# bluecher31/mlff-preconditioner

Hardware: AMD Instinct MI355X
Metric: CG iters/sec + GB/s on N×N fp64 kernel mat-vec; iters-to-1e-6 vs CPU ref (higher is better)
Workload: dtype f64

## Files before the change

### mlff-preconditioner_amd/csrc/common.h

```cpp
#pragma once

#include <hip/hip_runtime.h>
#include <rccl/rccl.h>

#include <cstdint>
#include <memory>
#include <string>
#include <cstdlib>
#include <vector>

#include "../../include/mlffpcg.h"

namespace mlff {

constexpr int kWave = 64;
constexpr int kBlock = 256;
constexpr int kPad = 64;
constexpr int kMaxPart = 1024;
constexpr int kVecGrid = 512;
constexpr int kSymTile = 512;

__host__ __device__ inline int64_t round_up(int64_t a, int64_t b) { return (a + b - 1) / b * b; }

enum : int { ST_RUNNING = 0, ST_RECHECK = 1, ST_CONVERGED = 2, ST_MAXITER = 3, ST_FAULT = 4 };

struct DevState {
  double rho, rho1, alpha, pq, rr, resid, atol, pad0;
  long long iters;
  long long maxiter;
  int status;
  int linalg_err;
  int pivot_err;
  int pad1;
  long long m_pi;
  double sqrt_piv;
  double best_val;
  long long best_pos;
  double rho_new;
};

constexpr int kSymGenMaxD = 3;
constexpr double kSymStreamRate = 5600.0;
constexpr double kSymGenRate = 5600.0;
constexpr int kSymThreeWgMinUnits = 2;
struct SymGen {
  const double *Xs = nullptr;
  int d = 0;
  double jitter = 0.0;
  int64_t N = 0, rows_per = 0, blk = 0;
  int n_s = 0;
  int qmode = 0;
  int roles = 0;
  int pool_first = 0;
  int wgs = 2;
};
enum SymRoles : int { kSymRolesCu = 0, kSymRolesIndex = 1, kSymRolesStream = 2, kSymRolesGen = 3 };
constexpr int kSymCuWords = 4096;

struct SymPack {
  bool ready = false;
  double *tiles = nullptr;
  int2 *list = nullptr;
  int64_t ntiles = 0;
  int64_t Np = 0;
  int64_t nb = 0;
  int64_t tiles_per_rank = 0;
  double *P = nullptr;
  int64_t nwhole = 0;
  int lsub = 2;
  int64_t pq_planes = 0;
  double *Pq = nullptr;
  unsigned char *split = nullptr;
  int *own = nullptr;
  int *plist = nullptr;
  int64_t pstride = 0;
  int pmax = 0;
  bool pq_ordered = false;
  int64_t t_split = 0;
  int64_t dyn = 0;
  int wgs = 0;
  bool rb4 = false;
  unsigned long long *ticket = nullptr;
  bool gen = false;
  SymGen gsrc;
  double *yg = nullptr;
  double *yr = nullptr;
  int64_t ystride = 0;
};

constexpr int kSymOwnSplit = 1 << 24;
constexpr int kSymPlistSlotBits = 16;
constexpr int kSymPlistMaxSlots = (1 << kSymPlistSlotBits) - 1;
__host__ __device__ inline int sym_own_entry(int slot, bool split) {
  return slot | (split ? kSymOwnSplit : 0);
}
__host__ __device__ inline int sym_own_slot(int e) { return e & (kSymOwnSplit - 1); }
__host__ __device__ inline bool sym_own_split(int e) { return (e & kSymOwnSplit) != 0; }
__host__ __device__ inline int sym_plist_entry(int slot, int plane) {
  return slot | (plane << kSymPlistSlotBits);
}
__host__ __device__ inline int sym_plist_slot(int e) { return e & kSymPlistMaxSlots; }
__host__ __device__ inline int sym_plist_plane(int e) { return e >> kSymPlistSlotBits; }

struct MfData {
  bool ready = false;
  int64_t M = 0, D = 0;
  int n = 0, n_perms = 0;
  double sig = 0.0;
// ... 612 lines not shown
```

### mlff-preconditioner_amd/csrc/kernels_sym.hip

```cpp
#include "common.h"

#include <algorithm>
#include <cstdlib>
#include <cstring>

namespace mlff {

typedef double d2 __attribute__((ext_vector_type(2)));

namespace {

constexpr int B = kSymTile;
constexpr int kRB = 8;
constexpr int kBatches = B / kRB;
constexpr int kTileRed = 6 * B;
constexpr int kTileLds = kTileRed + 4 * kRB * 64;
constexpr int kGenRowLds = kSymGenMaxD * B + B / 64;

__device__ __forceinline__ void decode_unit(long long u, int nwhole, int lsub, int &tile, int &h,
                                            int &gb0, int &gb1) {
  if (u < nwhole) {
    tile = (int)u;
    h = 0;
    gb0 = 0;
// ... 4 lines not shown
    h = (int)(q & ((1 << lsub) - 1));
    gb0 = h * (kBatches >> lsub);
    gb1 = gb0 + (kBatches >> lsub);
  }
}

__device__ __forceinline__ double gathered_rho(const PGather &pg, double *sh) {
  double v = 0.0;
  const int np = pg.world * kVecGrid;
  int f = threadIdx.x;
  for (; f + 7 * 256 < np; f += 8 * 256) {
    double t[8];
#pragma unroll
    for (int u = 0; u < 8; ++u) {
      const int g = f + u * 256;
      t[u] = pg.gb[(int64_t)(g / kVecGrid) * pg.gstride + pg.blk + (g % kVecGrid)];
    }
#pragma unroll
    for (int u = 0; u < 8; ++u) v += t[u];
  }
  for (; f < np; f += 256) v += pg.gb[(int64_t)(f / kVecGrid) * pg.gstride + pg.blk + (f % kVecGrid)];
  v = block_sum256(v, sh);
  __syncthreads();
  if (threadIdx.x == 0) sh[4] = v;
  __syncthreads();
  const double rho = sh[4];
  __syncthreads();
  return rho;
}

__device__ __forceinline__ double pg_z(const PGather &pg, int64_t i) {
  const int64_t rk = i / pg.blk;
  return rk < pg.world ? pg.gb[rk * pg.gstride + i % pg.blk] : 0.0;
}
__device__ __forceinline__ double pg_val(const PGather &pg, const double *v, int64_t i, double beta) {
  return pg.it > 1 ? fma(beta, v[i], pg_z(pg, i)) : pg_z(pg, i);
}
__device__ __forceinline__ d2 pg_val2(const PGather &pg, const double *v, int64_t i, double beta) {
  if (pg.gb == nullptr) return *reinterpret_cast<const d2 *>(v + i);
  const int64_t rk = i / pg.blk;
  const d2 z = rk < pg.world ? *reinterpret_cast<const d2 *>(pg.gb + rk * pg.gstride + i % pg.blk)
                             : d2{0.0, 0.0};
  if (pg.it <= 1) return z;
  const d2 po = *reinterpret_cast<const d2 *>(v + i);
  return d2{fma(beta, po.x, z.x), fma(beta, po.y, z.y)};
}

__device__ __forceinline__ double fused_p_beta(const PGather &pg, double rho, double *publish) {
  const double beta = pg.it > 1 ? rho / pg.st->rho1 : 0.0;
  if (blockIdx.x == 0 && threadIdx.x == 0) *publish = rho;
  return beta;
}

constexpr int kTicketWords = 4;
__device__ __forceinline__ void reset_work_counters(unsigned long long *ticket) {
  ticket[0] = 0ull;
  ticket[2] = 0ull;
  ticket[3] = 0ull;
}

struct UnitQueue {
  unsigned long long *c0, *c1, *c2;
  long long base0, hi0, base1, hi1, base2, hi2;
  int stage;
};
__device__ __forceinline__ bool take_unit(unsigned long long *c, long long base, long long hi,
                                          long long &u) {
  if (base >= hi) return false;
  u = base + (long long)atomicAdd(c, 1ull);
  return u < hi;
}
__device__ __forceinline__ long long next_unit(UnitQueue &q, long long nunits) {
  long long u;
  if (q.stage == 0) {
    if (take_unit(q.c0, q.base0, q.hi0, u)) return u;
    q.stage = 1;
  }
  if (q.stage == 1) {
    if (take_unit(q.c1, q.base1, q.hi1, u)) return u;
    q.stage = 2;
  }
  if (q.stage == 2) {
    if (take_unit(q.c2, q.base2, q.hi2, u)) return u;
    q.stage = 3;
  }
  return nunits;
}

__device__ __forceinline__ bool gen_index(const SymGen &gs, int64_t pos, int64_t &g) {
  const int64_t off = pos % gs.blk;
  g = (pos / gs.blk) * gs.rows_per + off;
  return off < gs.rows_per && g < gs.N;
}

struct GenCols {
  double x[8][kSymGenMaxD];
  unsigned valid;
};
__device__ __forceinline__ void gen_load_cols(const SymGen &gs, int J, int lane, GenCols &gc) {
  gc.valid = 0u;
#pragma unroll
  for (int j = 0; j < 8; ++j) {
    int64_t g;
    const bool ok = gen_index(gs, (int64_t)J * B + 2 * (lane + 64 * (j >> 1)) + (j & 1), g);
    if (ok) gc.valid |= 1u << j;
#pragma unroll
    for (int t = 0; t < kSymGenMaxD; ++t) gc.x[j][t] = (ok && t < gs.d) ? gs.Xs[g * gs.d + t] : 0.0;
  }
}
__device__ __forceinline__ bool gen_row_inside(const double *xrow, int r) {
  const unsigned *mask = reinterpret_cast<const unsigned *>(xrow + kSymGenMaxD * B);
  return ((mask[r >> 5] >> (r & 31)) & 1u) != 0u;
}
__device__ __forceinline__ void gen_stage_rows(const SymGen &gs, int I, int r0, int nr,
                                               double *__restrict__ xrow) {
  unsigned *mask = reinterpret_cast<unsigned *>(xrow + kSymGenMaxD * B);
  for (int i = threadIdx.x; i < nr; i += 256) {
    int64_t g;
    const bool ok = gen_index(gs, (int64_t)I * B + r0 + i, g);
#pragma unroll
    for (int t = 0; t < kSymGenMaxD; ++t)
      xrow[kSymGenMaxD * (r0 + i) + t] = (ok && t < gs.d) ? gs.Xs[g * gs.d + t] : 0.0;
    const unsigned long long m = __ballot(ok);
    if ((threadIdx.x & 63) == 0) {
      mask[(r0 + i) >> 5] = (unsigned)m;
      if (nr - i > 32) mask[((r0 + i) >> 5) + 1] = (unsigned)(m >> 32);
    }
  }
}
__device__ __forceinline__ bool gen_block_full(const SymGen &gs, int Jb) {
  int64_t g;
  const int64_t p0 = (int64_t)Jb * B, p1 = p0 + B - 1;
  return p0 / gs.blk == p1 / gs.blk && gen_index(gs, p0, g) && gen_index(gs, p1, g);
}
template <bool PLAIN, bool DIAG>
__device__ __forceinline__ void gen_row(const SymGen &gs, const GenCols &gc,
                                        const double *__restrict__ xrow, int r, int lane,
                                        d2 (&ar)[4]) {
// ... 36 lines not shown

template <bool GEN, bool PLAIN, bool DIAG, int RB>
__device__ __forceinline__ void tile_batch(d2 (&a)[GEN ? 1 : RB][4], const double *A,
                                           const SymGen &gs,
                                           const GenCols &gc, const double *xrow,
                                           bool diag_rt, const d2 (&pc)[4],
                                           const double *vrow, int rbase, int lane,
                                           double *red, double *rows,
                                           d2 (&acc)[4]) {
  const bool diag = GEN ? DIAG : diag_rt;
#pragma unroll(GEN ? 2 : kRB)
  for (int rr = 0; rr < kRB; ++rr) {
    d2 ar[4];
    if constexpr (GEN) {
      gen_row<PLAIN, DIAG>(gs, gc, xrow, rbase + rr, lane, ar);
    } else {
      if constexpr (RB < kRB)
        if (rr == RB) tile_load_batch<RB>(A, rbase + RB, lane, a);
#pragma unroll
      for (int q = 0; q < 4; ++q) ar[q] = a[rr % RB][q];
    }
    double s0 = ar[0].x * pc[0].x;
    double s1 = ar[0].y * pc[0].y;
#pragma unroll
    for (int q = 1; q < 4; ++q) {
      s0 = fma(ar[q].x, pc[q].x, s0);
      s1 = fma(ar[q].y, pc[q].y, s1);
    }
    red[rr * 64 + lane] = s0 + s1;
    if (!diag) {
      const double pr = vrow[rbase + rr];
#pragma unroll
      for (int q = 0; q < 4; ++q) {
        acc[q].x = fma(ar[q].x, pr, acc[q].x);
        acc[q].y = fma(ar[q].y, pr, acc[q].y);
      }
    }
  }
  __builtin_amdgcn_fence(__ATOMIC_RELEASE, "wavefront");
  __builtin_amdgcn_wave_barrier();
  __builtin_amdgcn_fence(__ATOMIC_ACQUIRE, "wavefront");
  const d2 *rp = reinterpret_cast<const d2 *>(red + (lane >> 3) * 64 + (lane & 7) * 8);
  const d2 t0 = rp[0], t1 = rp[1], t2 = rp[2], t3 = rp[3];
  double tt = ((t0.x + t0.y) + (t1.x + t1.y)) + ((t2.x + t2.y) + (t3.x + t3.y));
  tt += __shfl_xor(tt, 1, 64);
  tt += __shfl_xor(tt, 2, 64);
  tt += __shfl_xor(tt, 4, 64);
  if ((lane & 7) == 0) rows[rbase + (lane >> 3)] = tt;
  __builtin_amdgcn_fence(__ATOMIC_RELEASE, "wavefront");
  __builtin_amdgcn_wave_barrier();
  __builtin_amdgcn_fence(__ATOMIC_ACQUIRE, "wavefront");
}

template <bool GEN, bool PLAIN, bool DIAG, int RB>
__device__ __forceinline__ void tile_batches(d2 (&a)[GEN ? 1 : RB][4], const double *A,
                                             const SymGen &gs, const GenCols &gc, const double *xrow,
                                             bool diag_rt, const d2 (&pc)[4], const double *vrow,
                                             int gb0, int gb1, int w, int lane, double *red,
                                             double *rows, d2 (&acc)[4]) {
#pragma unroll 1
  for (int g = gb0 + w; g < gb1; g += 4) {
    if constexpr (!GEN)
      if (g != gb0 + w) tile_load_batch<RB>(A, g * kRB, lane, a);
    tile_batch<GEN, PLAIN, DIAG, RB>(a, A, gs, gc, xrow, diag_rt, pc, vrow, g * kRB, lane, red, rows,
                                     acc);
  }
}
template <bool GEN, int RB>
__device__ __forceinline__ void tile_unit(d2 (&a)[GEN ? 1 : RB][4], const double *A,
                                          const SymGen &gs, const GenCols &gc, const double *xrow,
                                          bool plain, bool diag, const d2 (&pc)[4],
                                          const double *vrow, int gb0, int gb1, int w, int lane,
                                          double *red, double *rows, d2 (&acc)[4]) {
  if (GEN && plain)
    tile_batches<GEN, GEN, false, RB>(a, A, gs, gc, xrow, diag, pc, vrow, gb0, gb1, w, lane, red, rows, acc);
  else if (GEN && diag)
    tile_batches<GEN, false, GEN, RB>(a, A, gs, gc, xrow, diag, pc, vrow, gb0, gb1, w, lane, red, rows, acc);
  else
    tile_batches<GEN, false, false, RB>(a, A, gs, gc, xrow, diag, pc, vrow, gb0, gb1, w, lane, red, rows, acc);
}

__device__ __forceinline__ void tile_stage_cols(const d2 (&acc)[4], double *cs, int w, int lane) {
  d2 *cs2 = reinterpret_cast<d2 *>(cs);
#pragma unroll
  for (int q = 0; q < 4; ++q) cs2[w * (B / 2) + lane + 64 * q] = acc[q];
}

__device__ __forceinline__ void tile_store_slots(double *P, double *Pq,
                                                 int64_t Np, int nb, int2 t, int h, int gb0, int gb1,
                                                 bool diag, const double *sh) {
  const double *rows = sh + B, *cs = sh + 2 * B;
  const int row0 = gb0 * kRB, nr = (gb1 - gb0) * kRB;
  double *Prow = P + (int64_t)t.y * Np + (int64_t)t.x * B + row0;
  for (int c = threadIdx.x; c < nr; c += 256) __builtin_nontemporal_store(rows[row0 + c], Prow + c);
  if (!diag) {
    double *Pc = h == 0 ? P : Pq + (int64_t)(h - 1) * nb * Np;
    double *Pcol = Pc + (int64_t)t.x * Np + (int64_t)t.y * B;
    for (int c = threadIdx.x; c < B; c += 256)
      __builtin_nontemporal_store((cs[c] + cs[B + c]) + (cs[2 * B + c] + cs[3 * B + c]), Pcol + c);
  }
}

__global__ __launch_bounds__(256) void k_symv_tiles(const double *__restrict__ tiles,
                                                    const int2 *__restrict__ list,
                                                    const double *__restrict__ v,
                                                    double *__restrict__ P,
                                                    double *__restrict__ Pq, int64_t Np,
                                                    int nwhole, int nb, int lsub,
                                                    const int *__restrict__ status) {
  if (status != nullptr && *status != ST_RUNNING) return;
  __shared__ double sh[kTileLds];
  const int lane = threadIdx.x & 63, w = threadIdx.x >> 6;
  int tile, h, gb0, gb1;
  decode_unit(blockIdx.x, nwhole, lsub, tile, h, gb0, gb1);
  const int2 t = list[tile];
  const double *A = tiles + (int64_t)tile * B * B;
  d2 pc[4], a[kRB][4];
#pragma unroll
  for (int q = 0; q < 4; ++q)
    pc[q] = *reinterpret_cast<const d2 *>(v + (int64_t)t.y * B + 2 * (lane + 64 * q));
  tile_load_batch<kRB>(A, (int64_t)(gb0 + w) * kRB, lane, a);
  for (int i = gb0 * kRB + threadIdx.x; i < gb1 * kRB; i += 256) sh[i] = v[(int64_t)t.x * B + i];
  __syncthreads();
  const bool diag = t.x == t.y;
  const GenCols none{};
  d2 acc[4];
#pragma unroll
  for (int q = 0; q < 4; ++q) acc[q] = d2{0.0, 0.0};
  tile_unit<false, kRB>(a, A, SymGen{}, none, nullptr, false, diag, pc, sh, gb0, gb1, w, lane,
                   sh + kTileRed + w * kRB * 64, sh + B, acc);
  if (!diag) tile_stage_cols(acc, sh + 2 * B, w, lane);
  __syncthreads();
  tile_store_slots(P, Pq, Np, nb, t, h, gb0, gb1, diag, sh);
}

struct SymvArgs {
  const double *tiles;
  const int2 *list;
  const double *v;
  double *P, *Pq;
  int64_t Np;
  int nwhole;
  long long nunits;
  int nb, lsub;
  PGather pg;
  double beta;
};

template <bool GEN, int RB>
__device__ __forceinline__ long long symv_units(const SymvArgs &k, const SymGen &gs, long long u,
                                                UnitQueue q, double *__restrict__ sh,
                                                long long *s_next) {
  const int lane = threadIdx.x & 63, w = threadIdx.x >> 6;
  double *vrow = sh, *rows = sh + B, *cs = sh + 2 * B;
  double *red = sh + kTileRed + w * kRB * 64;
  double *xrow = sh + kTileLds;
  const PGather &pg = k.pg;
  const double *v = k.v;
  const double beta = k.beta;
  long long units_done = 0;
  int tile, h, gb0, gb1;
  decode_unit(u, k.nwhole, k.lsub, tile, h, gb0, gb1);
  int2 t = k.list[tile];
  const double *A = k.tiles + (int64_t)tile * B * B;
  d2 pc[4], a[GEN ? 1 : RB][4];
  GenCols gc;
#pragma unroll
  for (int q = 0; q < 4; ++q) pc[q] = pg_val2(pg, v, (int64_t)t.y * B + 2 * (lane + 64 * q), beta);
  if constexpr (!GEN) tile_load_batch<RB>(A, (int64_t)(gb0 + w) * kRB, lane, a);
  if (threadIdx.x == 0) *s_next = next_unit(q, k.nunits);
  for (int i = threadIdx.x; i < (gb1 - gb0) * kRB; i += 256) {
    const int64_t gi = (int64_t)t.x * B + gb0 * kRB + i;
    vrow[gb0 * kRB + i] = pg.gb != nullptr ? pg_val(pg, v, gi, beta) : v[gi];
  }
  if (GEN) {
    gen_stage_rows(gs, t.x, gb0 * kRB, (gb1 - gb0) * kRB, xrow);
    gen_load_cols(gs, t.y, lane, gc);
  }
  __syncthreads();
  while (true) {
    const bool diag = t.x == t.y;
    const bool plain = GEN && !diag && gen_block_full(gs, t.x) && gen_block_full(gs, t.y);
    d2 acc[4];
#pragma unroll
    for (int q = 0; q < 4; ++q) acc[q] = d2{0.0, 0.0};
    tile_unit<GEN, RB>(a, A, gs, gc, xrow, plain, diag, pc, vrow, gb0, gb1, w, lane, red, rows, acc);
    if (!diag) tile_stage_cols(acc, cs, w, lane);
    __syncthreads();
    const long long un = *s_next;
    int tile2 = 0, h2 = 0, gb02 = 0, gb12 = 0;
    int2 t2 = t;
    const double *A2 = A;
    if (un < k.nunits) {
      decode_unit(un, k.nwhole, k.lsub, tile2, h2, gb02, gb12);
      t2 = k.list[tile2];
      A2 = k.tiles + (int64_t)tile2 * B * B;
#pragma unroll
      for (int q = 0; q < 4; ++q)
        pc[q] = pg_val2(pg, v, (int64_t)t2.y * B + 2 * (lane + 64 * q), beta);
      if constexpr (GEN)
        gen_load_cols(gs, t2.y, lane, gc);
      else
        tile_load_batch<RB>(A2, (int64_t)(gb02 + w) * kRB, lane, a);
    }
    tile_store_slots(k.P, k.Pq, k.Np, k.nb, t, h, gb0, gb1, diag, sh);
    __syncthreads();
    ++units_done;
    if (un >= k.nunits) break;
    if (threadIdx.x == 0) *s_next = next_unit(q, k.nunits);
    tile = tile2;
    h = h2;
    gb0 = gb02;
    gb1 = gb12;
    t = t2;
    A = A2;
    for (int i = threadIdx.x; i < (gb1 - gb0) * kRB; i += 256) {
      const int64_t gi = (int64_t)t.x * B + gb0 * kRB + i;
      vrow[gb0 * kRB + i] = pg.gb != nullptr ? pg_val(pg, v, gi, beta) : v[gi];
    }
    if (GEN) gen_stage_rows(gs, t.x, gb0 * kRB, (gb1 - gb0) * kRB, xrow);
    __syncthreads();
  }
  return units_done;
}

__device__ __forceinline__ unsigned cu_key() {
  unsigned xcc = 0, hw = 0;
  asm volatile("s_getreg_b32 %0, hwreg(HW_REG_XCC_ID)" : "=s"(xcc));
  asm volatile("s_getreg_b32 %0, hwreg(HW_REG_HW_ID)" : "=s"(hw));
  return ((xcc & 0xfu) << 8) | ((hw >> 8) & 0xffu);
}

constexpr int kTraceWords = 4;

template <bool ROLES, int RB = kRB>
__global__ __launch_bounds__(256, RB < kRB ? 3 : 1) void k_symv_dyn(const double *__restrict__ tiles,
                                                  const int2 *__restrict__ list,
                                                  const double *__restrict__ v,
                                                  double *__restrict__ P,
                                                  double *__restrict__ Pq, int64_t Np,
                                                  int nwhole, long long nunits, int nb,
                                                  int lsub,
                                                  unsigned long long *__restrict__ ticket,
                                                  const int *__restrict__ status, PGather pg,
                                                  SymGen gs,
                                                  unsigned long long *wgtrace = nullptr) {
  if (status != nullptr && *status != ST_RUNNING) return;
  unsigned long long *tr = wgtrace != nullptr ? wgtrace + kTraceWords * blockIdx.x : nullptr;
  if (tr != nullptr && threadIdx.x == 0) tr[0] = wall_clock64();
  __shared__ double sh[kTileLds + (ROLES ? kGenRowLds : 0)];
  __shared__ long long s_next;
  __shared__ int s_role;
  if (!ROLES && (long long)blockIdx.x >= nunits) return;
  if (ROLES && threadIdx.x == 0) {
    int r = gs.roles == kSymRolesGen ? 1 : 0;
    const unsigned wgs = (unsigned)gs.wgs;
    if (gs.roles == kSymRolesIndex) r = blockIdx.x % wgs != 0u;
    if (gs.roles == kSymRolesCu) r = atomicAdd(ticket + kTicketWords + cu_key(), 1ull) % wgs != 0ull;
    s_role = r;
  }
  if (!ROLES && tr != nullptr && threadIdx.x == 0) tr[3] = 1ull | (unsigned long long)cu_key() << 2;
  const double beta = pg.gb != nullptr ? fused_p_beta(pg, gathered_rho(pg, sh), &pg.st->rho_new) : 0.0;
  UnitQueue q{ticket, ticket, ticket, (long long)gridDim.x, nunits, 0, 0, 0, 0, 0};
  long long u = blockIdx.x;
  bool gen = false;
  if (ROLES) {
    __syncthreads();
    gen = __builtin_amdgcn_readfirstlane(s_role) != 0;
    const bool pool_first = gs.pool_first != 0 && gs.qmode != (gen ? 1 : 2);
    unsigned long long *cs = ticket, *cg = ticket + 2, *cq = ticket + 3;
    const long long ns = gs.n_s;
    q.c0 = gen ? cg : cs;
    q.base0 = gen ? ns : 0;
    q.hi0 = gen ? nwhole : ns;
    unsigned long long *co = gen ? cs : cg;
    const long long olo = gen ? 0 : ns, ohi = gen ? ns : nwhole;
    q.c1 = pool_first ? cq : co;
    q.base1 = pool_first ? nwhole : olo;
    q.hi1 = pool_first ? nunits : ohi;
    q.c2 = pool_first ? co : cq;
    q.base2 = pool_first ? olo : nwhole;
    q.hi2 = pool_first ? ohi : nunits;
    if (threadIdx.x == 0) {
      s_next = next_unit(q, nunits);
      if (tr != nullptr) tr[3] = 1ull | (gen ? 2ull : 0ull) | (unsigned long long)cu_key() << 2;
    }
    __syncthreads();
    u = s_next;
    __syncthreads();
    if (u >= nunits) {
      if (tr != nullptr && threadIdx.x == 0) tr[1] = wall_clock64();
      return;
    }
  }
  const SymvArgs k{tiles, list, v, P, Pq, Np, nwhole, nunits, nb, lsub, pg, beta};
  long long units_done;
  if constexpr (ROLES) {
    if (gen)
      units_done = symv_units<true, RB>(k, gs, u, q, sh, &s_next);
    else
      units_done = symv_units<false, RB>(k, gs, u, q, sh, &s_next);
  } else {
    units_done = symv_units<false, RB>(k, gs, u, q, sh, &s_next);
  }
  if (tr != nullptr && threadIdx.x == 0) {
    tr[1] = wall_clock64();
    tr[2] = (unsigned long long)units_done;
  }
}

template <bool EPI, bool PQ>
__global__ __launch_bounds__(256) void k_sym_reduce(const double *__restrict__ P,
                                                    const double *__restrict__ Pq,
                                                    const unsigned char *__restrict__ split,
                                                    int t_split, int64_t Np, int nb, int nq,
                                                    int64_t n_out, double *__restrict__ y,
                                                    double sigma, double lam,
                                                    const double *__restrict__ vloc,
                                                    double *__restrict__ pq_part,
                                                    unsigned long long *__restrict__ ticket,
                                                    const int *__restrict__ status,
                                                    PGather pg = PGather{},
                                                    double *pw = nullptr) {
  if (status != nullptr && *status != ST_RUNNING) return;
  if (blockIdx.x == 0 && threadIdx.x == 0) reset_work_counters(ticket);
  double apq = 0.0;
  const double beta = PQ && pg.gb != nullptr ? fused_p_beta(pg, pg.st->rho_new, &pg.st->rho) : 0.0;
  const int64_t pl = (int64_t)nb * Np;
  for (int64_t i = (int64_t)blockIdx.x * 256 + threadIdx.x; i < n_out;
       i += (int64_t)gridDim.x * 256) {
    const int bi = (int)(i / B);
    double s = 0.0;
    const int tend = t_split > bi ? t_split : bi + 1;
    const int t8 = tend < nb ? tend : nb;
    int t = 0;
    for (; t + 15 < t8; t += 16) {
      double v[16];
#pragma unroll
      for (int u = 0; u < 16; ++u) v[u] = __builtin_nontemporal_load(P + (int64_t)(t + u) * Np + i);
#pragma unroll
      for (int u = 0; u < 16; ++u) s += v[u];
    }
    for (; t + 7 < t8; t += 8) {
      double v[8];
#pragma unroll
      for (int u = 0; u < 8; ++u) v[u] = __builtin_nontemporal_load(P + (int64_t)(t + u) * Np + i);
#pragma unroll
      for (int u = 0; u < 8; ++u) s += v[u];
    }
    for (; t < nb; t += 8) {
      double v[8];
#pragma unroll
      for (int u = 0; u < 8; ++u) {
        v[u] = 0.0;
        const int tu = t + u;
        if (tu < nb) {
          v[u] = P[(int64_t)tu * Np + i];
          if (tu > bi && split[(int64_t)tu * nb + bi])
            for (int hq = 0; hq < nq; ++hq) v[u] += Pq[hq * pl + (int64_t)tu * Np + i];
// ... 345 lines not shown
  int64_t gc[2];
  bool vc[2];
#pragma unroll
  for (int h = 0; h < 2; ++h) {
    const int64_t pos = (int64_t)t.y * B + threadIdx.x + 256 * h;
    const int64_t off = pos % blk;
    gc[h] = (pos / blk) * rows_per + off;
    vc[h] = off < rows_per && gc[h] < N;
#pragma unroll
    for (int u = 0; u < 8; ++u) xc[h][u] = (vc[h] && u < d) ? Xs[gc[h] * d + u] : 0.0;
  }
  for (int r = 0; r < B; ++r) {
    const int64_t pos = (int64_t)t.x * B + r;
    const int64_t off = pos % blk;
    const int64_t gr = (pos / blk) * rows_per + off;
    const bool vr = off < rows_per && gr < N;
#pragma unroll
    for (int h = 0; h < 2; ++h) {
      double val = 0.0;
      if (vr && vc[h]) val = (gr == gc[h]) ? 1.0 + jitter : rbf_value(xc[h], Xs, gr, d);
      __builtin_nontemporal_store(val, T + (int64_t)r * B + threadIdx.x + 256 * h);
    }
  }
}

__global__ __launch_bounds__(256) void k_rbf_exp_probe(const double *__restrict__ s, int64_t n,
                                                       double *__restrict__ lib_out,
                                                       double *__restrict__ lean_out) {
  for (int64_t i = (int64_t)blockIdx.x * 256 + threadIdx.x; i < n; i += (int64_t)gridDim.x * 256) {
    lib_out[i] = rbf_of_sqdist(s[i]);
    lean_out[i] = rbf_of_sqdist_lean(s[i]);
  }
}

}

void launch_rbf_exp_probe(const double *s, int64_t n, double *lib_out, double *lean_out,
                          hipStream_t st) {
  if (n <= 0) return;
  const unsigned grid = (unsigned)std::min<int64_t>((n + 255) / 256, 4096);
  hipLaunchKernelGGL(k_rbf_exp_probe, dim3(grid), dim3(256), 0, st, s, n, lib_out, lean_out);
}

struct SymKnobs {
  int64_t whole_rounds = -1;
  int lsub = 2;
  bool dynamic = true;
  bool gen = true;
  int64_t gen_tiles = -1;
  int gen_quarters = 0;
  int roles = kSymRolesCu;
  int pool_first = 0;
  int wgs = 0;
  bool reduce_list = true;
  bool pq_ordered = false;
  long long trace_at = 0;
};

static SymKnobs sym_knobs() {
  SymKnobs k;
  if (const char *e = std::getenv("MLFF_SYM_WHOLE_ROUNDS")) k.whole_rounds = std::max<int64_t>(0, std::atoll(e));
  if (const char *e = std::getenv("MLFF_SYM_LSUB")) {
    const int v = std::atoi(e);
    if (v >= 1 && v <= 4) k.lsub = v;
  }
  if (const char *e = std::getenv("MLFF_SYM_SCHED")) k.dynamic = std::strcmp(e, "static") != 0;
  if (const char *e = std::getenv("MLFF_SYM_GEN")) k.gen = std::atoi(e) != 0;
  if (const char *e = std::getenv("MLFF_SYM_GEN_TILES")) k.gen_tiles = std::max<int64_t>(0, std::atoll(e));
  if (const char *e = std::getenv("MLFF_SYM_GEN_QUARTERS")) {
    const int v = std::atoi(e);
    if (v >= 0 && v <= 2) k.gen_quarters = v;
  }
  if (const char *e = std::getenv("MLFF_SYM_ROLES")) {
    if (std::strcmp(e, "index") == 0) k.roles = kSymRolesIndex;
    if (std::strcmp(e, "stream") == 0) k.roles = kSymRolesStream;
    if (std::strcmp(e, "gen") == 0) k.roles = kSymRolesGen;
  }
  if (const char *e = std::getenv("MLFF_SYM_STEAL")) k.pool_first = std::strcmp(e, "pool") == 0;
  if (const char *e = std::getenv("MLFF_SYM_WGS")) {
    const int v = std::atoi(e);
    if (v == 2 || v == 3) k.wgs = v;
  }
  if (const char *e = std::getenv("MLFF_SYM_REDUCE_LIST")) k.reduce_list = std::atoi(e) != 0;
  if (const char *e = std::getenv("MLFF_SYM_PQ_ORDERED")) k.pq_ordered = std::atoi(e) != 0;
  if (const char *e = std::getenv("MLFF_SYM_TRACE")) k.trace_at = std::atoll(e);
  return k;
}

static void print_symv_trace(const unsigned long long *tr, unsigned G, int64_t units, int wgs,
                             hipStream_t s) {
  std::vector<unsigned long long> h((size_t)kTraceWords * G);
  if (hipStreamSynchronize(s) != hipSuccess ||
      hipMemcpy(h.data(), tr, sizeof(unsigned long long) * h.size(), hipMemcpyDeviceToHost) != hipSuccess)
    return;
  unsigned long long t0 = ~0ull, t1 = 0;
  std::vector<double> st, en, un;
  for (unsigned g = 0; g < G; ++g) {
    const unsigned long long *r = &h[(size_t)kTraceWords * g];
    if (r[0] == 0) continue;
    t0 = std::min(t0, r[0]);
    t1 = std::max(t1, r[1]);
  }
  double idle = 0.0;
  std::vector<int> cu_s(kSymCuWords, 0), cu_g(kSymCuWords, 0);
  int xs[16] = {0}, xg[16] = {0};
  double un_s = 0.0, un_g = 0.0;
  for (unsigned g = 0; g < G; ++g) {
    const unsigned long long *r = &h[(size_t)kTraceWords * g];
    if (r[0] == 0) continue;
    st.push_back(10.0 * (double)(r[0] - t0));
    en.push_back(10.0 * (double)(r[1] - t0));
    un.push_back((double)r[2]);
    idle += 10.0 * (double)(t1 - r[1]) + 10.0 * (double)(r[0] - t0);
    if (!(r[3] & 1ull)) continue;
    const bool gen = (r[3] & 2ull) != 0;
    const unsigned key = (unsigned)(r[3] >> 2) & (kSymCuWords - 1);
    ++(gen ? cu_g : cu_s)[key];
    ++(gen ? xg : xs)[key >> 8];
    (gen ? un_g : un_s) += (double)r[2];
  }
  auto q = [](std::vector<double> v, double f) {
    std::sort(v.begin(), v.end());
    return v.empty() ? 0.0 : v[(size_t)(f * (double)(v.size() - 1))];
  };
  const double span = 10.0 * (double)(t1 - t0);
  std::fprintf(stderr,
               "[sym trace] units %lld on %zu workgroups (units per wg p0/p50/p100 %.0f/%.0f/%.0f); "
               "span %.1f us; starts p50/p100 %.1f/%.1f us; ends p0/p10/p50/p90/p100 "
               "%.1f/%.1f/%.1f/%.1f/%.1f us; idle (ramp + tail) %.1f %% of wg-time\n",
               (long long)units, st.size(), q(un, 0.0), q(un, 0.5), q(un, 1.0), 1e-3 * span,
               1e-3 * q(st, 0.5), 1e-3 * q(st, 1.0), 1e-3 * q(en, 0.0), 1e-3 * q(en, 0.1),
               1e-3 * q(en, 0.5), 1e-3 * q(en, 0.9), 1e-3 * q(en, 1.0),
               100.0 * idle / (span * (double)st.size()));
  int cus = 0, paired = 0, two_s = 0, two_g = 0, other = 0;
  for (int k = 0; k < kSymCuWords; ++k) {
    if (cu_s[k] + cu_g[k] == 0) continue;
    ++cus;
    if (cu_s[k] == 1 && cu_g[k] == wgs - 1)
      ++paired;
    else if (cu_s[k] == wgs && cu_g[k] == 0)
      ++two_s;
    else if (cu_s[k] == 0 && cu_g[k] == wgs)
      ++two_g;
    else
      ++other;
  }
  std::string per_xcc;
  for (int x = 0; x < 16; ++x)
    if (xs[x] + xg[x] > 0)
      per_xcc += " " + std::to_string(x) + ":" + std::to_string(xs[x]) + "s+" + std::to_string(xg[x]) + "g";
  std::fprintf(stderr,
               "[sym trace] roles: %d distinct CU keys; CUs holding {1 stream + %d gen} %d, {%d stream} "
               "%d, {%d gen} %d, other %d; units taken stream / gen %.0f / %.0f (%.0f / %.0f per ms "
               "of the span); per XCC id%s\n",
               cus, wgs - 1, paired, wgs, two_s, wgs, two_g, other, un_s, un_g, 1e6 * un_s / span,
               1e6 * un_g / span, per_xcc.c_str());
}

void launch_symv(const SymPack &sp, const double *v_full, double *P, const int *status,
                 hipStream_t s, PGather pg) {
  if (sp.ntiles == 0) return;
  const int64_t grid = sp.nwhole + ((sp.ntiles - sp.nwhole) << sp.lsub);
  if (sp.dyn == 0) {
    hipLaunchKernelGGL(k_symv_tiles, dim3((unsigned)grid), dim3(256), 0, s, sp.tiles, sp.list, v_full,
                       P, sp.Pq, sp.Np, (int)sp.nwhole, (int)sp.nb, sp.lsub, status);
    return;
  }
  const unsigned G = (unsigned)std::min<int64_t>(sp.dyn, grid);
  static const long long trace_at = sym_knobs().trace_at;
  static long long launches = 0;
  unsigned long long *tr = nullptr;
  if (trace_at > 0 && ++launches == trace_at &&
      hipMalloc(&tr, sizeof(unsigned long long) * kTraceWords * G) == hipSuccess)
    (void)hipMemsetAsync(tr, 0, sizeof(unsigned long long) * kTraceWords * G, s);
  if (sp.gen && sp.rb4)
    hipLaunchKernelGGL((k_symv_dyn<true, 4>), dim3(G), dim3(256), 0, s,
                       sp.tiles, sp.list, v_full, P, sp.Pq, sp.Np, (int)sp.nwhole, (long long)grid,
                       (int)sp.nb, sp.lsub, sp.ticket, status, pg, sp.gsrc, tr);
  else if (sp.gen)
    hipLaunchKernelGGL(k_symv_dyn<true>, dim3(G), dim3(256), 0, s,
                       sp.tiles, sp.list, v_full, P, sp.Pq, sp.Np, (int)sp.nwhole, (long long)grid,
                       (int)sp.nb, sp.lsub, sp.ticket, status, pg, sp.gsrc, tr);
  else
    hipLaunchKernelGGL(k_symv_dyn<false>, dim3(G), dim3(256), 0, s,
                       sp.tiles, sp.list, v_full, P, sp.Pq, sp.Np, (int)sp.nwhole, (long long)grid,
                       (int)sp.nb, sp.lsub, sp.ticket, status, pg, SymGen{}, tr);
// ... 77 lines not shown
  const int a = I / tpr, c = J / tpr;
  if (a == c) return a;
  return ((I + J) & 1) ? a : c;
}


struct SymPlan {
  int64_t Np = 0;
  int nb = 0, tpr = 0;
  std::vector<int2> list;
  std::vector<unsigned char> trans;
  int64_t nt = 0, nwhole = 0;
  int lsub = 2;
  int64_t nq = 3;
  int64_t dyn = 0;
  int wgs = 2;
  bool rb4 = false;
  bool gen = false;
  SymGen gsrc;
};

static SymPlan sym_plan(const mlff_ctx *ctx, const SymKnobs &kn) {
  SymPlan pl;
  pl.Np = round_up(ctx->ld, B);
  pl.nb = (int)(pl.Np / B);
  pl.tpr = ctx->world > 1 ? (int)(ctx->blk / B) : pl.nb;
  for (int I = 0; I < pl.nb; ++I)
    for (int J = 0; J <= I; ++J) {
      if (owner_host(I, J, pl.tpr) != ctx->rank) continue;
      pl.list.push_back(make_int2(I, J));
      pl.trans.push_back(ctx->world > 1 && (I / pl.tpr) != ctx->rank ? 1 : 0);
    }
  pl.nt = (int64_t)pl.list.size();
  int cus = 0;
  if (hipDeviceGetAttribute(&cus, hipDeviceAttributeMultiprocessorCount, ctx->device) != hipSuccess ||
      cus < 1)
    cus = 256;
  const int64_t C = 2 * (int64_t)cus;
  pl.nwhole = (pl.nt / C) * C;
  if (kn.whole_rounds >= 0) pl.nwhole = std::min<int64_t>(pl.nwhole, kn.whole_rounds * C);
  pl.lsub = kn.lsub;
  pl.nq = ((int64_t)1 << pl.lsub) - 1;
  pl.dyn = kn.dynamic ? C : 0;
  if (pl.dyn > 0 && pl.nt > 0 && !ctx->has_matrix && ctx->rbf.ready && ctx->rbf.d >= 1 &&
      ctx->rbf.d <= kSymGenMaxD) {
    int64_t n_s = (int64_t)((double)pl.nwhole * kSymStreamRate / (kSymStreamRate + kSymGenRate) + 0.5);
    if (kn.gen_tiles >= 0) n_s = pl.nwhole - std::min<int64_t>(pl.nwhole, kn.gen_tiles);
    const int qmode = kn.gen_quarters;
    bool on = kn.gen;
    if (pl.nwhole == pl.nt && n_s == pl.nwhole) on = false;
    if (n_s == pl.nwhole && qmode == 1) on = false;
    if (on) {
      pl.gen = true;
      if (kn.wgs != 2) {
        int occ = 0;
        if (hipOccupancyMaxActiveBlocksPerMultiprocessor(&occ, k_symv_dyn<true, 4>, 256, 0) != hipSuccess ||
            occ < 1)
          occ = 2;
        const int64_t nunits = pl.nwhole + ((pl.nt - pl.nwhole) << pl.lsub);
        pl.rb4 = kn.wgs == 3 || (occ > 2 && nunits >= kSymThreeWgMinUnits * occ * cus);
        if (pl.rb4) {
          pl.wgs = occ;
          pl.dyn = (int64_t)occ * cus;
        }
      }
      pl.gsrc = SymGen{ctx->rbf.Xs, ctx->rbf.d, ctx->rbf.jitter, ctx->N, ctx->rows_per, ctx->blk,
                       (int)n_s, qmode, kn.roles, kn.pool_first, pl.wgs};
    }
  }
  return pl;
}

static int sym_alloc(mlff_ctx *ctx, const SymPlan &pl, const SymKnobs &kn) {
  SymPack &sp = ctx->sym;
  hipStream_t s = ctx->stream;
  const int64_t nt = pl.nt, nb = pl.nb, Np = pl.Np, nq = pl.nq;
  if (sp.tiles == nullptr || sp.ntiles != nt || sp.Np != Np || sp.pq_planes != nq) {
    sym_free(sp);
    if (nt > 0) {
      MLFF_HIP(ctx, hipMalloc(&sp.tiles, sizeof(double) * nt * B * B));
      MLFF_HIP(ctx, hipMalloc(&sp.list, sizeof(int2) * nt));
    }
    MLFF_HIP(ctx, hipMalloc(&sp.P, sizeof(double) * nb * Np));
    MLFF_HIP(ctx, hipMemsetAsync(sp.P, 0, sizeof(double) * nb * Np, s));
    MLFF_HIP(ctx, hipMalloc(&sp.Pq, sizeof(double) * nq * nb * Np));
    MLFF_HIP(ctx, hipMemsetAsync(sp.Pq, 0, sizeof(double) * nq * nb * Np, s));
    sp.pq_planes = nq;
    MLFF_HIP(ctx, hipMalloc(&sp.split, (size_t)nb * nb));
    MLFF_HIP(ctx, hipMalloc(&sp.own, sizeof(int) * (size_t)nb * (nb + 1)));
    const size_t tw = (kTicketWords + kSymCuWords) * sizeof(unsigned long long);
    MLFF_HIP(ctx, hipMalloc(&sp.ticket, tw));
    MLFF_HIP(ctx, hipMemsetAsync(sp.ticket, 0, tw, s));
    if (ctx->world > 1) {
      sp.ystride = ctx->blk + round_up(ctx->world, kPad);
      const int64_t ny = (int64_t)ctx->world * sp.ystride;
      MLFF_HIP(ctx, hipMalloc(&sp.yg, sizeof(double) * ny));
      MLFF_HIP(ctx, hipMalloc(&sp.yr, sizeof(double) * sp.ystride));
      MLFF_HIP(ctx, hipMemsetAsync(sp.yg, 0, sizeof(double) * ny, s));
      MLFF_HIP(ctx, hipMemsetAsync(sp.yr, 0, sizeof(double) * sp.ystride, s));
    }
  }
  sp.ntiles = nt;
  sp.Np = Np;
  sp.nb = nb;
  sp.tiles_per_rank = pl.tpr;
  sp.nwhole = pl.nwhole;
  sp.lsub = pl.lsub;
  sp.dyn = pl.dyn;
  sp.wgs = pl.dyn > 0 ? pl.wgs : 0;
  sp.rb4 = pl.rb4;
  sp.gen = pl.gen;
  sp.gsrc = pl.gsrc;
  sp.pq_ordered = kn.pq_ordered;
  return MLFF_OK;
}

static int sym_slot_tables(mlff_ctx *ctx, const SymPlan &pl, const SymKnobs &kn) {
  SymPack &sp = ctx->sym;
  hipStream_t s = ctx->stream;
  const int nb = pl.nb;
// ... 101 lines not shown
```

Before: 625.1.

## Defer next-unit claim to last batch and lower three-workgroup threshold

The dynamic symmetric mat-vec scheduler now claims its next work unit late, during the final batch of the current tile, instead of at tile start. This keeps units from being reserved early by workgroups that will not reach them for a while, which should reduce tail imbalance. It also lowers the unit-count threshold for switching to three workgroups per CU when late commit is on, and adds an optional endgame rule (off by default) where generator workgroups decline whole tiles near the end. A per-wave lambda call and extra trace instrumentation are added; the late claim may expose atomic latency at the tile boundary.

```diff
diff --git a/mlff-preconditioner_amd/csrc/common.h b/mlff-preconditioner_amd/csrc/common.h
--- a/mlff-preconditioner_amd/csrc/common.h
+++ b/mlff-preconditioner_amd/csrc/common.h
@@ -7,6 +7,7 @@
 #include <memory>
 #include <string>
 #include <cstdlib>
+#include <cstring>
 #include <vector>
 
 #include "../../include/mlffpcg.h"
@@ -42,7 +43,7 @@
 constexpr int kSymGenMaxD = 3;
 constexpr double kSymStreamRate = 5600.0;
 constexpr double kSymGenRate = 5600.0;
-constexpr int kSymThreeWgMinUnits = 2;
+constexpr double kSymThreeWgMinUnits = 1.375;
 struct SymGen {
   const double *Xs = nullptr;
   int d = 0;
@@ -53,7 +54,27 @@
   int roles = 0;
   int pool_first = 0;
   int wgs = 2;
-};
+  int late = 0;
+  int endgame = 0;
+};
+constexpr double kSymEndgameRounds = 0.0;
+constexpr bool kSymLateCommit = true;
+inline void sym_parse_commit(const char *e, bool &late) {
+  if (e == nullptr) return;
+  if (std::strcmp(e, "early") == 0) late = false;
+  if (std::strcmp(e, "late") == 0) late = true;
+}
+inline void sym_parse_endgame(const char *e, double &rounds) {
+  if (e == nullptr) return;
+  char *end = nullptr;
+  const double v = std::strtod(e, &end);
+  if (end != e && v >= 0.0 && v <= 1e9) rounds = v;
+}
+inline int sym_endgame_theta(double rounds, int64_t workgroups, int wgs) {
+  if (!(rounds > 0.0) || wgs < 1) return 0;
+  const double t = rounds * (double)(workgroups / wgs) + 0.5;
+  return t >= 2147483647.0 ? 2147483647 : (int)t;
+}
 enum SymRoles : int { kSymRolesCu = 0, kSymRolesIndex = 1, kSymRolesStream = 2, kSymRolesGen = 3 };
 constexpr int kSymCuWords = 4096;
 
diff --git a/mlff-preconditioner_amd/csrc/kernels_sym.hip b/mlff-preconditioner_amd/csrc/kernels_sym.hip
--- a/mlff-preconditioner_amd/csrc/kernels_sym.hip
+++ b/mlff-preconditioner_amd/csrc/kernels_sym.hip
@@ -80,17 +80,25 @@
   return beta;
 }
 
-constexpr int kTicketWords = 4;
+constexpr int kTicketWords = 6;
+constexpr int kTicketPresent = 4;
 __device__ __forceinline__ void reset_work_counters(unsigned long long *ticket) {
   ticket[0] = 0ull;
   ticket[2] = 0ull;
   ticket[3] = 0ull;
-}
+  ticket[kTicketPresent] = 0ull;
+}
+
+constexpr int kTraceWords = 10;
+enum : int { kTrEmpty = 4, kTrDecline = 5, kTrLast = 6, kTrCyc0 = 7, kTrCyc1 = 8, kTrDry = 9 };
 
 struct UnitQueue {
   unsigned long long *c0, *c1, *c2;
   long long base0, hi0, base1, hi1, base2, hi2;
   int stage;
+  const unsigned long long *ticket;
+  int theta;
+  unsigned long long *tr;
 };
 __device__ __forceinline__ bool take_unit(unsigned long long *c, long long base, long long hi,
                                           long long &u) {
@@ -98,20 +106,40 @@
   u = base + (long long)atomicAdd(c, 1ull);
   return u < hi;
 }
+__device__ __forceinline__ unsigned long long counter_now(const unsigned long long *c) {
+  return __hip_atomic_load(c, __ATOMIC_RELAXED, __HIP_MEMORY_SCOPE_AGENT);
+}
+__device__ __forceinline__ bool endgame_declines(const UnitQueue &q) {
+  if (q.theta <= 0 || q.stage > 2) return false;
+  if (counter_now(q.ticket + kTicketPresent) == 0ull) return false;
+  const unsigned long long ts = counter_now(q.ticket), tg = counter_now(q.ticket + 2);
+  const long long n_s = q.base0, n_g = q.hi0 - q.base0;
+  const long long left = (n_s - (long long)min(ts, (unsigned long long)n_s)) +
+                         (n_g - (long long)min(tg, (unsigned long long)n_g));
+  return left <= q.theta;
+}
+__device__ __forceinline__ void trace_once(unsigned long long *tr, int word) {
+  if (tr != nullptr && tr[word] == 0ull) tr[word] = wall_clock64();
+}
+__device__ __forceinline__ bool take_range(UnitQueue &q, int r, unsigned long long *c,
+                                           long long base, long long hi, bool decline,
+                                           long long &u) {
+  if (q.stage != r) return false;
+  if (!(decline && c != q.ticket + 3)) {
+    if (take_unit(c, base, hi, u)) return true;
+    if (base < hi) trace_once(q.tr, kTrEmpty);
+  }
+  q.stage = r + 1;
+  return false;
+}
 __device__ __forceinline__ long long next_unit(UnitQueue &q, long long nunits) {
   long long u;
-  if (q.stage == 0) {
-    if (take_unit(q.c0, q.base0, q.hi0, u)) return u;
-    q.stage = 1;
-  }
-  if (q.stage == 1) {
-    if (take_unit(q.c1, q.base1, q.hi1, u)) return u;
-    q.stage = 2;
-  }
-  if (q.stage == 2) {
-    if (take_unit(q.c2, q.base2, q.hi2, u)) return u;
-    q.stage = 3;
-  }
+  const bool decline = endgame_declines(q);
+  if (decline) trace_once(q.tr, kTrDecline);
+  if (take_range(q, 0, q.c0, q.base0, q.hi0, decline, u)) return u;
+  if (take_range(q, 1, q.c1, q.base1, q.hi1, decline, u)) return u;
+  if (take_range(q, 2, q.c2, q.base2, q.hi2, decline, u)) return u;
+  trace_once(q.tr, kTrDry);
   return nunits;
 }
 
@@ -254,32 +282,33 @@
   __builtin_amdgcn_fence(__ATOMIC_ACQUIRE, "wavefront");
 }
 
-template <bool GEN, bool PLAIN, bool DIAG, int RB>
+template <bool GEN, bool PLAIN, bool DIAG, int RB, class Last>
 __device__ __forceinline__ void tile_batches(d2 (&a)[GEN ? 1 : RB][4], const double *A,
                                              const SymGen &gs, const GenCols &gc, const double *xrow,
                                              bool diag_rt, const d2 (&pc)[4], const double *vrow,
                                              int gb0, int gb1, int w, int lane, double *red,
-                                             double *rows, d2 (&acc)[4]) {
+                                             double *rows, d2 (&acc)[4], Last &last) {
 #pragma unroll 1
   for (int g = gb0 + w; g < gb1; g += 4) {
     if constexpr (!GEN)
       if (g != gb0 + w) tile_load_batch<RB>(A, g * kRB, lane, a);
+    if (g + 4 >= gb1) last();
     tile_batch<GEN, PLAIN, DIAG, RB>(a, A, gs, gc, xrow, diag_rt, pc, vrow, g * kRB, lane, red, rows,
                                      acc);
   }
 }
-template <bool GEN, int RB>
+template <bool GEN, int RB, class Last>
 __device__ __forceinline__ void tile_unit(d2 (&a)[GEN ? 1 : RB][4], const double *A,
                                           const SymGen &gs, const GenCols &gc, const double *xrow,
                                           bool plain, bool diag, const d2 (&pc)[4],
                                           const double *vrow, int gb0, int gb1, int w, int lane,
-                                          double *red, double *rows, d2 (&acc)[4]) {
+                                          double *red, double *rows, d2 (&acc)[4], Last &last) {
   if (GEN && plain)
-    tile_batches<GEN, GEN, false, RB>(a, A, gs, gc, xrow, diag, pc, vrow, gb0, gb1, w, lane, red, rows, acc);
+    tile_batches<GEN, GEN, false, RB>(a, A, gs, gc, xrow, diag, pc, vrow, gb0, gb1, w, lane, red, rows, acc, last);
   else if (GEN && diag)
-    tile_batches<GEN, false, GEN, RB>(a, A, gs, gc, xrow, diag, pc, vrow, gb0, gb1, w, lane, red, rows, acc);
+    tile_batches<GEN, false, GEN, RB>(a, A, gs, gc, xrow, diag, pc, vrow, gb0, gb1, w, lane, red, rows, acc, last);
   else
-    tile_batches<GEN, false, false, RB>(a, A, gs, gc, xrow, diag, pc, vrow, gb0, gb1, w, lane, red, rows, acc);
+    tile_batches<GEN, false, false, RB>(a, A, gs, gc, xrow, diag, pc, vrow, gb0, gb1, w, lane, red, rows, acc, last);
 }
 
 __device__ __forceinline__ void tile_stage_cols(const d2 (&acc)[4], double *cs, int w, int lane) {
@@ -329,8 +358,9 @@
   d2 acc[4];
 #pragma unroll
   for (int q = 0; q < 4; ++q) acc[q] = d2{0.0, 0.0};
+  auto nothing = [] {};
   tile_unit<false, kRB>(a, A, SymGen{}, none, nullptr, false, diag, pc, sh, gb0, gb1, w, lane,
-                   sh + kTileRed + w * kRB * 64, sh + B, acc);
+                   sh + kTileRed + w * kRB * 64, sh + B, acc, nothing);
   if (!diag) tile_stage_cols(acc, sh + 2 * B, w, lane);
   __syncthreads();
   tile_store_slots(P, Pq, Np, nb, t, h, gb0, gb1, diag, sh);
@@ -347,6 +377,8 @@
   int nb, lsub;
   PGather pg;
   double beta;
+  bool late;
+  unsigned long long *tr;
 };
 
 template <bool GEN, int RB>
@@ -370,7 +402,12 @@
 #pragma unroll
   for (int q = 0; q < 4; ++q) pc[q] = pg_val2(pg, v, (int64_t)t.y * B + 2 * (lane + 64 * q), beta);
   if constexpr (!GEN) tile_load_batch<RB>(A, (int64_t)(gb0 + w) * kRB, lane, a);
-  if (threadIdx.x == 0) *s_next = next_unit(q, k.nunits);
+  const bool late = k.late;
+  auto commit = [&] {
+    if (late && threadIdx.x == 0) *s_next = next_unit(q, k.nunits);
+  };
+  if (!late && threadIdx.x == 0) *s_next = next_unit(q, k.nunits);
+  if (k.tr != nullptr && threadIdx.x == 0) k.tr[kTrLast] = wall_clock64();
   for (int i = threadIdx.x; i < (gb1 - gb0) * kRB; i += 256) {
     const int64_t gi = (int64_t)t.x * B + gb0 * kRB + i;
     vrow[gb0 * kRB + i] = pg.gb != nullptr ? pg_val(pg, v, gi, beta) : v[gi];
@@ -386,7 +423,8 @@
     d2 acc[4];
 #pragma unroll
     for (int q = 0; q < 4; ++q) acc[q] = d2{0.0, 0.0};
-    tile_unit<GEN, RB>(a, A, gs, gc, xrow, plain, diag, pc, vrow, gb0, gb1, w, lane, red, rows, acc);
+    tile_unit<GEN, RB>(a, A, gs, gc, xrow, plain, diag, pc, vrow, gb0, gb1, w, lane, red, rows, acc,
+                       commit);
     if (!diag) tile_stage_cols(acc, cs, w, lane);
     __syncthreads();
     const long long un = *s_next;
@@ -409,7 +447,8 @@
     __syncthreads();
     ++units_done;
     if (un >= k.nunits) break;
-    if (threadIdx.x == 0) *s_next = next_unit(q, k.nunits);
+    if (!late && threadIdx.x == 0) *s_next = next_unit(q, k.nunits);
+    if (k.tr != nullptr && threadIdx.x == 0) k.tr[kTrLast] = wall_clock64();
     tile = tile2;
     h = h2;
     gb0 = gb02;
@@ -432,8 +471,6 @@
   asm volatile("s_getreg_b32 %0, hwreg(HW_REG_HW_ID)" : "=s"(hw));
   return ((xcc & 0xfu) << 8) | ((hw >> 8) & 0xffu);
 }
-
-constexpr int kTraceWords = 4;
 
 template <bool ROLES, int RB = kRB>
 __global__ __launch_bounds__(256, RB < kRB ? 3 : 1) void k_symv_dyn(const double *__restrict__ tiles,
@@ -449,7 +486,10 @@
                                                   unsigned long long *wgtrace = nullptr) {
   if (status != nullptr && *status != ST_RUNNING) return;
   unsigned long long *tr = wgtrace != nullptr ? wgtrace + kTraceWords * blockIdx.x : nullptr;
-  if (tr != nullptr && threadIdx.x == 0) tr[0] = wall_clock64();
+  if (tr != nullptr && threadIdx.x == 0) {
+    tr[0] = wall_clock64();
+    tr[kTrCyc0] = __builtin_amdgcn_s_memtime();
+  }
   __shared__ double sh[kTileLds + (ROLES ? kGenRowLds : 0)];
   __shared__ long long s_next;
   __shared__ int s_role;
@@ -463,7 +503,8 @@
   }
   if (!ROLES && tr != nullptr && threadIdx.x == 0) tr[3] = 1ull | (unsigned long long)cu_key() << 2;
   const double beta = pg.gb != nullptr ? fused_p_beta(pg, gathered_rho(pg, sh), &pg.st->rho_new) : 0.0;
-  UnitQueue q{ticket, ticket, ticket, (long long)gridDim.x, nunits, 0, 0, 0, 0, 0};
+  UnitQueue q{ticket, ticket, ticket, (long long)gridDim.x, nunits, 0, 0, 0, 0, 0,
+              ticket, 0, tr};
   long long u = blockIdx.x;
   bool gen = false;
   if (ROLES) {
@@ -483,7 +524,10 @@
     q.c2 = pool_first ? co : cq;
     q.base2 = pool_first ? olo : nwhole;
     q.hi2 = pool_first ? ohi : nunits;
+    q.theta = gen ? gs.endgame : 0;
     if (threadIdx.x == 0) {
+      if (!gen)
+        __hip_atomic_store(ticket + kTicketPresent, 1ull, __ATOMIC_RELAXED, __HIP_MEMORY_SCOPE_AGENT);
       s_next = next_unit(q, nunits);
       if (tr != nullptr) tr[3] = 1ull | (gen ? 2ull : 0ull) | (unsigned long long)cu_key() << 2;
     }
@@ -491,11 +535,14 @@
     u = s_next;
     __syncthreads();
     if (u >= nunits) {
-      if (tr != nullptr && threadIdx.x == 0) tr[1] = wall_clock64();
+      if (tr != nullptr && threadIdx.x == 0) {
+        tr[1] = wall_clock64();
+        tr[kTrCyc1] = __builtin_amdgcn_s_memtime();
+      }
       return;
     }
   }
-  const SymvArgs k{tiles, list, v, P, Pq, Np, nwhole, nunits, nb, lsub, pg, beta};
+  const SymvArgs k{tiles, list, v, P, Pq, Np, nwhole, nunits, nb, lsub, pg, beta, gs.late != 0, tr};
   long long units_done;
   if constexpr (ROLES) {
     if (gen)
@@ -507,6 +554,7 @@
   }
   if (tr != nullptr && threadIdx.x == 0) {
     tr[1] = wall_clock64();
+    tr[kTrCyc1] = __builtin_amdgcn_s_memtime();
     tr[2] = (unsigned long long)units_done;
   }
 }
@@ -958,6 +1006,8 @@
   int roles = kSymRolesCu;
   int pool_first = 0;
   int wgs = 0;
+  bool late = kSymLateCommit;
+  double endgame = kSymEndgameRounds;
   bool reduce_list = true;
   bool pq_ordered = false;
   long long trace_at = 0;
@@ -987,6 +1037,8 @@
     const int v = std::atoi(e);
     if (v == 2 || v == 3) k.wgs = v;
   }
+  sym_parse_commit(std::getenv("MLFF_SYM_COMMIT"), k.late);
+  sym_parse_endgame(std::getenv("MLFF_SYM_ENDGAME"), k.endgame);
   if (const char *e = std::getenv("MLFF_SYM_REDUCE_LIST")) k.reduce_list = std::atoi(e) != 0;
   if (const char *e = std::getenv("MLFF_SYM_PQ_ORDERED")) k.pq_ordered = std::atoi(e) != 0;
   if (const char *e = std::getenv("MLFF_SYM_TRACE")) k.trace_at = std::atoll(e);
@@ -1038,6 +1090,34 @@
                1e-3 * q(st, 0.5), 1e-3 * q(st, 1.0), 1e-3 * q(en, 0.0), 1e-3 * q(en, 0.1),
                1e-3 * q(en, 0.5), 1e-3 * q(en, 0.9), 1e-3 * q(en, 1.0),
                100.0 * idle / (span * (double)st.size()));
+  double dry = -1.0, empty = -1.0, declined_first = -1.0;
+  int declined = 0;
+  std::vector<double> en_r[2], last_r[2], mhz_r[2];
+  for (unsigned g = 0; g < G; ++g) {
+    const unsigned long long *r = &h[(size_t)kTraceWords * g];
+    if (r[0] == 0) continue;
+    auto at = [&](int w) { return 10.0 * (double)(r[w] - t0); };
+    if (r[kTrEmpty] != 0 && (empty < 0.0 || at(kTrEmpty) < empty)) empty = at(kTrEmpty);
+    if (r[kTrDecline] != 0) {
+      ++declined;
+      if (declined_first < 0.0 || at(kTrDecline) < declined_first) declined_first = at(kTrDecline);
+    } else if (r[kTrDry] != 0 && (dry < 0.0 || at(kTrDry) < dry)) {
+      dry = at(kTrDry);
+    }
+    const int role = (r[3] & 2ull) != 0 ? 1 : 0;
+    en_r[role].push_back(at(1));
+    if (r[kTrLast] != 0) last_r[role].push_back(at(kTrLast));
+    if (r[1] > r[0]) mhz_r[role].push_back(100.0 * (double)(r[kTrCyc1] - r[kTrCyc0]) / (double)(r[1] - r[0]));
+  }
+  std::fprintf(stderr,
+               "[sym trace] end: counters dry at %.1f us, first range empty at %.1f us; %d workgroups "
+               "declined a whole tile (first at %.1f us); ends p50/p100 stream %.1f/%.1f gen %.1f/%.1f us; "
+               "last unit started p50/p100 stream %.1f/%.1f gen %.1f/%.1f us; in-kernel clock stream / "
+               "gen %.0f / %.0f MHz\n",
+               1e-3 * dry, 1e-3 * empty, declined, 1e-3 * declined_first, 1e-3 * q(en_r[0], 0.5),
+               1e-3 * q(en_r[0], 1.0), 1e-3 * q(en_r[1], 0.5), 1e-3 * q(en_r[1], 1.0),
+               1e-3 * q(last_r[0], 0.5), 1e-3 * q(last_r[0], 1.0), 1e-3 * q(last_r[1], 0.5),
+               1e-3 * q(last_r[1], 1.0), q(mhz_r[0], 0.5), q(mhz_r[1], 0.5));
   int cus = 0, paired = 0, two_s = 0, two_g = 0, other = 0;
   for (int k = 0; k < kSymCuWords; ++k) {
     if (cu_s[k] + cu_g[k] == 0) continue;
@@ -1221,20 +1301,22 @@
     if (n_s == pl.nwhole && qmode == 1) on = false;
     if (on) {
       pl.gen = true;
+      const double min_units = kn.late ? kSymThreeWgMinUnits : 2.0;
       if (kn.wgs != 2) {
         int occ = 0;
         if (hipOccupancyMaxActiveBlocksPerMultiprocessor(&occ, k_symv_dyn<true, 4>, 256, 0) != hipSuccess ||
             occ < 1)
           occ = 2;
         const int64_t nunits = pl.nwhole + ((pl.nt - pl.nwhole) << pl.lsub);
-        pl.rb4 = kn.wgs == 3 || (occ > 2 && nunits >= kSymThreeWgMinUnits * occ * cus);
+        pl.rb4 = kn.wgs == 3 || (occ > 2 && (double)nunits >= min_units * occ * cus);
         if (pl.rb4) {
           pl.wgs = occ;
           pl.dyn = (int64_t)occ * cus;
         }
       }
       pl.gsrc = SymGen{ctx->rbf.Xs, ctx->rbf.d, ctx->rbf.jitter, ctx->N, ctx->rows_per, ctx->blk,
-                       (int)n_s, qmode, kn.roles, kn.pool_first, pl.wgs};
+                       (int)n_s, qmode, kn.roles, kn.pool_first, pl.wgs, kn.late ? 1 : 0,
+                       sym_endgame_theta(kn.endgame, pl.dyn, pl.wgs)};
     }
   }
   return pl;
```

Result: no change. 628.1, median of 6 (+0.5%).
